# gildas-lormeau/zlib-streams-ts

Measured on AMD Instinct MI355X. Metric: uncompressed MB/s, deflate-raw L6, 4096x64KiB batch at 1/2/4/8 GPUs, higher is better.
Workload: dtype u8; 1 GPU; 4096 x 65536 B text-corpus streams split across the GPUs, deflate-raw level 6; global_streams=4096, streams_per_gpu=4096, stream_bytes=65536, level=6, format=deflate-raw, compressed_bytes=91855591, parallelism=dp1

## Files before the change

zlib-streams-ts_amd/csrc/deflate_parse.hip:

```cpp
#include <hip/hip_runtime.h>
#include <type_traits>
#include "zs_common.h"
#include "zs_kernels.h"
#include "zs_parse.h"

template <uint32_t SEG>
struct zs_seg_cfg {
  static constexpr uint32_t SPEC = (SEG + 260u + 3u) & ~3u;
  static constexpr uint32_t SYNC = SEG + 4u;
  static constexpr uint32_t FIX = SPEC;
  static constexpr uint32_t WORDS = SPEC + SYNC + FIX;
};
static_assert(zs_seg_cfg<ZS_PARSE_SEG>::WORDS == ZS_PARSE_SEG_WORDS, "scratch layout shared with capi.cpp");
static_assert(zs_seg_cfg<ZS_PARSE2W_SEG>::WORDS == ZS_PARSE2W_SEG_WORDS, "scratch layout shared with capi.cpp");
static_assert(zs_seg_cfg<ZS_PARSE4W_SEG>::WORDS == ZS_PARSE4W_SEG_WORDS, "scratch layout shared with capi.cpp");

#define ZS_WAVE_SYNC()                                   \
  do {                                                   \
    __builtin_amdgcn_fence(__ATOMIC_SEQ_CST, "workgroup"); \
    __builtin_amdgcn_wave_barrier();                     \
  } while (0)

struct zs_round_state {
  zs_pstate t;
  uint32_t total, last_sym;
};

template <uint32_t WIN>
struct zs_parse_win {
  uint4 m[WIN / 2][64];
};
template <>
struct zs_parse_win<0> {};

struct zs_seg_tab {
  uint32_t off[65];
  uint32_t nf[64];
  uint32_t from[64];
};

template <uint32_t WIN>
union zs_parse_lds {
  zs_parse_win<WIN> W;
  zs_seg_tab T;
};

static __device__ __forceinline__ uint32_t zs_sym_len(uint32_t v) {
  return (v & 0x80000000u) ? ((v >> 16) & 0xffu) + ZS_MIN_MATCH : 1u;
}
static __device__ __forceinline__ zs_pstate zs_read_state(const zs_pstate& x, uint32_t l) {
  zs_pstate r;
  r.p = (uint32_t)__builtin_amdgcn_readlane((int)x.p, (int)l);
  r.ma = (uint32_t)__builtin_amdgcn_readlane((int)x.ma, (int)l);
  r.ml = (uint32_t)__builtin_amdgcn_readlane((int)x.ml, (int)l);
  r.ms = (uint32_t)__builtin_amdgcn_readlane((int)x.ms, (int)l);
  return r;
}

#ifndef ZS_PARSE_PROF
#define ZS_PARSE_PROF 0
#endif
#if ZS_PARSE_PROF
__device__ unsigned long long zs_pp_stat[16];
extern "C" int zs_parse_stats(unsigned long long* out) {
  return (int)hipMemcpyFromSymbol(out, HIP_SYMBOL(zs_pp_stat), sizeof(zs_pp_stat));
}
#define PP_T(v) unsigned long long v = wall_clock64()
#define PP_ACC(i, v) do { if ((threadIdx.x & 63u) == 0) atomicAdd(&zs_pp_stat[i], wall_clock64() - v); } while (0)
#else
#define PP_T(v) do { } while (0)
#define PP_ACC(i, v) do { } while (0)
#endif

#define ZS_GATHER 16
#ifndef ZS_PARSE_WIN
#define ZS_PARSE_WIN 32
#endif


template <uint32_t WIN, uint32_t SEG, uint32_t NWV, bool DICT, bool FILT>
static __device__ __forceinline__ void zs_parse_body(zs_parse_win<WIN>& W, zs_seg_tab& T, zs_round_state& RS,
                                                     const uint8_t* __restrict__ in,
                                                     const uint64_t* __restrict__ in_off,
                                                     const uint32_t* __restrict__ in_len,
                                                     const uint64_t* __restrict__ pos_base,
                                                     const uint32_t* __restrict__ blk_base,
                                                     const uint2* __restrict__ mres, uint32_t* __restrict__ syms,
                                                     zs_block* __restrict__ blocks, zs_stream* __restrict__ streams,
                                                     uint32_t* __restrict__ scratch, int good, int lazy,
                                                     const uint32_t* __restrict__ dstart ZS_PAR_ARG) {
  using CF = zs_seg_cfg<SEG>;
  const int s = blockIdx.x;
  const uint32_t lane = threadIdx.x & 63u, wave = threadIdx.x >> 6;
  const uint32_t n = in_len[s];
  const uint32_t p0 = DICT ? dstart[s] : 0u;
  const uint8_t* src = in + in_off[s];
  const uint2* M = mres + pos_base[s];
  uint32_t* sy = syms + pos_base[s] + s;
  uint32_t* scr = scratch + (size_t)CF::WORDS * (pos_base[s] / SEG + s + 64u * wave);
  zs_block* blk = blocks + blk_base[s];
  const uint32_t nseg = (n - p0 + SEG - 1) / SEG;
  const bool aligned = ((uintptr_t)src & 3u) == 0;

  zs_pstate t = {p0, 0, ZS_MIN_MATCH - 1, 0};
  uint32_t total = 0;
  uint32_t last_sym = 0;
  if (NWV > 1) {
    if (threadIdx.x == 0) RS = {t, 0u, 0u};
    __syncthreads();
  }

  for (uint32_t sr = 0; sr < nseg; sr += 64u * NWV) {
    const uint32_t r0 = sr + 64u * wave;
    const uint32_t nr = r0 < nseg ? min(64u, nseg - r0) : 0u;
    const bool mine = lane < nr;
    const uint32_t a = mine ? p0 + (r0 + lane) * SEG : n, b = mine ? min(n, a + SEG) : n;
    uint32_t* spec = scr + (size_t)lane * CF::WORDS;
    uint32_t* sync = spec + CF::SPEC;
    uint32_t* fix = sync + CF::SYNC;

    PP_T(tA);
    zs_pstate st = {a, 0, ZS_MIN_MATCH - 1, 0};
    uint32_t cnt = 0;
    {
      uint32_t nsync = 0;
      uint4 sacc = make_uint4(0, 0, 0, 0), yacc = make_uint4(0, 0, 0, 0);
      auto step = [&](uint2 e, uint32_t lit) __attribute__((always_inline)) {
        if (st.ml == ZS_MIN_MATCH - 1) {
          const uint32_t y = ((st.p - a) << 17) | (st.ma << 16) | cnt, m = nsync & 3u;
          yacc.x = m == 0 ? y : yacc.x;
          yacc.y = m == 1 ? y : yacc.y;
          yacc.z = m == 2 ? y : yacc.z;
          yacc.w = m == 3 ? y : yacc.w;
          if (++nsync % 4 == 0) *reinterpret_cast<uint4*>(sync + nsync - 4) = yacc;
        }
        const uint32_t v = zs_parse_step<FILT>(st, e, lit, n, good, lazy ZS_PAR_PASS);
        if (v != ZS_NONE) {
          const uint32_t m = cnt & 3u;
          sacc.x = m == 0 ? v : sacc.x;
          sacc.y = m == 1 ? v : sacc.y;
          sacc.z = m == 2 ? v : sacc.z;
          sacc.w = m == 3 ? v : sacc.w;
          if (++cnt % 4 == 0) *reinterpret_cast<uint4*>(spec + cnt - 4) = sacc;
        }
      };
      if constexpr (WIN == 0) {
        while (st.p < b) {
          const uint32_t p = st.p;
          step(M[p], p > 0 ? src[p - 1] : 0u);
        }
      } else {
        constexpr uint32_t NP = WIN / 2;
        const uint32_t c = lane & (NP - 1u), tg = lane & ~(NP - 1u);
        const uint4* g = reinterpret_cast<const uint4*>(M);
        const uint32_t glast = ((n + 7u) >> 1) & ~3u;
        const uint32_t* s4 = reinterpret_cast<const uint32_t*>(src);
        const uint32_t slast = (n - 1u) >> 2;
        const uint32_t cw = (c + 1u) >> 1;
        for (uint64_t staging; (staging = __ballot(st.p < b)) != 0;) {
          const uint32_t w = st.p & ~3u;
          auto stage = [&](auto al) __attribute__((always_inline)) {
            constexpr bool AL = decltype(al)::value;
            uint4 mv[NP];
            uint32_t sv[NP];
            const uint32_t act = (uint32_t)(staging >> tg) & ((1u << NP) - 1u);
            uint32_t tb = tg << 2, c7 = c & 7u;
            asm volatile("" : "+v"(tb), "+v"(c7));
#pragma unroll
            for (uint32_t r = 0; r < NP; r++) sv[r] = (uint32_t)__builtin_amdgcn_ds_bpermute((int)(tb + 4u * r), (int)w);
#pragma unroll
            for (uint32_t r = 0; r < NP; r++) {
              if ((act >> r) & 1u) {
                const uint32_t wt = sv[r];
                mv[r] = g[min(wt / 2 + c, glast - 1u)];
                if constexpr (AL) {
                  sv[r] = s4[min(max(wt / 4 + cw, 1u) - 1u, slast)];
                } else {
                  uint16_t h = 0;
                  if (n > 1) __builtin_memcpy(&h, src + min(max(wt + 2u * c, 1u), n - 1u) - 1u, 2);
                  sv[r] = n > 1 ? (uint32_t)h | ((wt | c) == 0 ? 0x10000u : 0u) : src[0] | 0x10000u;
                }
              }
            }
#pragma unroll
            for (uint32_t r = 0; r < NP; r++) {
              uint32_t l0, l1;
              if constexpr (AL) {
                const uint32_t nx = (uint32_t)__builtin_amdgcn_update_dpp(0, (int)sv[r], 0x101, 0xf, 0xf, false);
                l0 = (c & 1u) ? (sv[r] >> 8) & 0xffu : sv[r] >> 24;
                l1 = (c & 1u) ? (sv[r] >> 16) & 0xffu : nx & 0xffu;
              } else {
                l0 = sv[r] & 0xffu;
                l1 = (sv[r] >> 16) ? l0 : (sv[r] >> 8) & 0xffu;
              }
              mv[r].x |= l0 << 25;
              mv[r].y |= (l0 >> 7) << 31;
              mv[r].z |= l1 << 25;
              mv[r].w |= (l1 >> 7) << 31;
              if ((act >> r) & 1u) W.m[c][tg + (r ^ c7)] = mv[r];
            }
          };
          if (aligned) stage(std::true_type{}); else stage(std::false_type{});
          while (st.p < b && st.p < w + WIN) {
            const uint32_t o = st.p - w;
            const uint2 e = reinterpret_cast<const uint2*>(&W.m[o >> 1][lane ^ ((o >> 1) & 7u)])[o & 1];
            step(e, (e.x >> 25) | ((e.y >> 31) << 7));
          }
        }
      }
      if (mine) {
        for (uint32_t i = nsync & ~3u; i < nsync; i++) sync[i] = (i & 3u) == 0 ? yacc.x : (i & 3u) == 1 ? yacc.y : yacc.z;
        for (uint32_t i = cnt & ~3u; i < cnt; i++) spec[i] = (i & 3u) == 0 ? sacc.x : (i & 3u) == 1 ? sacc.y : sacc.z;
        sync[nsync] = ZS_NONE;
        if (b == n && st.ma) spec[cnt++] = src[n - 1];
      }
    }

    PP_ACC(0, tA);
    uint32_t nf = 0, from = ZS_NONE, start = 0, R = 0, tot0 = 0;
    bool final_lit_r = false;
    for (uint32_t k = 0; k < NWV + (NWV > 1 ? 1u : 0u); k++) {
    if (NWV > 1) __syncthreads();
    if (nr != 0 && k == wave) {
    PP_T(tB);
    if (NWV > 1) {
      t = RS.t;
      total = RS.total;
    }
    zs_pstate after;
    auto catch_up = [&](zs_pstate c) __attribute__((always_inline)) {
      uint32_t si = 0, sv = sync[0];
      uint4 facc = make_uint4(0, 0, 0, 0);
      nf = 0;
      from = ZS_NONE;
      start = c.p - c.ma;
      while (c.p < b) {
        if (c.ml == ZS_MIN_MATCH - 1) {
          const uint32_t key = ((c.p - a) << 1) | c.ma;
          while ((sv >> 16) < key) sv = sync[++si];
          if ((sv >> 16) == key) { from = sv & 0xffffu; break; }
        }
        const uint32_t p = c.p;
        const uint32_t v = zs_parse_step<FILT>(c, M[p], p > 0 ? src[p - 1] : 0u, n, good, lazy ZS_PAR_PASS);
        if (v != ZS_NONE) {
          const uint32_t m = nf & 3u;
          facc.x = m == 0 ? v : facc.x;
          facc.y = m == 1 ? v : facc.y;
          facc.z = m == 2 ? v : facc.z;
          facc.w = m == 3 ? v : facc.w;
          if (++nf % 4 == 0) *reinterpret_cast<uint4*>(fix + nf - 4) = facc;
        }
      }
      for (uint32_t i = nf & ~3u; i < nf; i++) fix[i] = (i & 3u) == 0 ? facc.x : (i & 3u) == 1 ? facc.y : facc.z;
      if (from == ZS_NONE && b == n && c.ma) fix[nf++] = src[n - 1];
      after = from != ZS_NONE ? st : c;
    };
    {
      zs_pstate e;
      const int up = (int)((lane + 63u) & 63u);
      e.p = (uint32_t)__shfl((int)st.p, up, 64);
      e.ma = (uint32_t)__shfl((int)st.ma, up, 64);
      e.ml = (uint32_t)__shfl((int)st.ml, up, 64);
      e.ms = (uint32_t)__shfl((int)st.ms, up, 64);
      if (lane == 0) e = t;
      if (mine) catch_up(e);
    }
    for (uint32_t j = 0; j < nr; j++) {
      if (j > 0 && (uint32_t)__builtin_amdgcn_readlane((int)from, (int)(j - 1)) == ZS_NONE) {
        if (lane == j) catch_up(t);
      }
      t = zs_read_state(after, j);
    }

    const uint32_t run = mine ? nf + (from == ZS_NONE ? 0u : cnt - from) : 0u;
    uint32_t incl = run;
#pragma unroll
    for (int d = 1; d < 64; d <<= 1) {
      const uint32_t y = __shfl_up(incl, d, 64);
      if (lane >= (uint32_t)d) incl += y;
    }
    R = (uint32_t)__builtin_amdgcn_readlane((int)incl, 63);
    T.off[lane] = incl - run;
    if (lane == 63) T.off[64] = R;
    T.nf[lane] = nf;
    T.from[lane] = from;
    tot0 = total;
    final_lit_r = r0 + nr == nseg && t.ma != 0;
    total += R;
    if (NWV > 1 && lane == 0) {
      RS.t = t;
      RS.total = total;
    }
    PP_ACC(1, tB);
    }
    if (nr != 0 && k == wave + (NWV > 1 ? 1u : 0u)) {
    ZS_WAVE_SYNC();
    PP_T(tC);
    uint32_t js = 0, lastv = 0;
    for (uint32_t g0 = 0; g0 < R; g0 += 64 * ZS_GATHER) {
      uint32_t v[ZS_GATHER];
#pragma unroll
      for (int k = 0; k < ZS_GATHER; k++) {
        const uint32_t g = g0 + 64 * k + lane;
        v[k] = 0;
        if (g < R) {
          while (T.off[js + 1] <= g) js++;
          const uint32_t i = g - T.off[js], nfj = T.nf[js];
          const uint32_t* base = scr + (size_t)js * CF::WORDS;
          v[k] = i < nfj ? base[CF::SPEC + CF::SYNC + i] : base[T.from[js] + i - nfj];
        }
      }
#pragma unroll
      for (int k = 0; k < ZS_GATHER; k++) {
        const uint32_t g = g0 + 64 * k + lane;
        if (g < R) sy[tot0 + g] = v[k];
        if (g == R - 1) lastv = v[k];
      }
    }
    if (R) {
      last_sym = (uint32_t)__shfl((int)lastv, (int)((R - 1) & 63u), 64);
      if (NWV > 1 && lane == 0) RS.last_sym = last_sym;
    }

    PP_ACC(2, tC);
    PP_T(tD);
    const uint32_t unchecked = final_lit_r ? tot0 + R - 1 : ZS_NONE;
    for (uint32_t gi = (tot0 / ZS_P_SYM_END + 1) * ZS_P_SYM_END - 1; gi < tot0 + R; gi += ZS_P_SYM_END) {
      if (gi == unchecked) continue;
      const uint32_t g = gi - tot0;
      uint32_t j = 0;
      while (T.off[j + 1] <= g) j++;
      const uint32_t i = g - T.off[j], nfj = T.nf[j], fj = T.from[j];
      const uint32_t* base = scr + (size_t)j * CF::WORDS;
      uint32_t acc = 0, li = 0;
      for (uint32_t q = lane; q <= i; q += 64) {
        const uint32_t l = zs_sym_len(q < nfj ? base[CF::SPEC + CF::SYNC + q] : base[fj + q - nfj]);
        acc += l;
        li = q == i ? l : li;
      }
#pragma unroll
      for (int d = 32; d >= 1; d >>= 1) {
        acc += __shfl_xor(acc, d, 64);
        li += __shfl_xor(li, d, 64);
      }
      const uint32_t end = (uint32_t)__builtin_amdgcn_readlane((int)start, (int)j) + acc;
      if (lane == 0) {
        const uint32_t bi = (gi + 1) / ZS_P_SYM_END - 1;
        blk[bi].in_end = end;
        blk[bi].pad = zs_slides(end - li + 1, n ZS_PAR_PASS);
      }
    }
    PP_ACC(3, tD);
    ZS_WAVE_SYNC();
    }
    }
  }
  if (NWV > 1) {
    __syncthreads();
    if (wave != 0) return;
    t = RS.t;
    total = RS.total;
    last_sym = RS.last_sym;
  }

  PP_T(tE);
  const bool final_lit = nseg > 0 && t.ma != 0;
  const uint32_t checked = final_lit ? total - 1 : total;
  const uint32_t nflush = checked / ZS_P_SYM_END;
  const uint32_t v_last = total == 0 ? 0u : final_lit ? n - 1 : n - zs_sym_len(last_sym) + 1;
  const uint32_t final_slides = zs_slides(v_last, n ZS_PAR_PASS);
  ZS_WAVE_SYNC();
  for (uint32_t b0 = 0; b0 <= nflush; b0 += 64) {
    const uint32_t b = b0 + lane;
    zs_block k;
    if (b <= nflush) {
      const uint32_t in_start = b == 0 ? p0 : blk[b - 1].in_end;
      const uint32_t in_end = b < nflush ? blk[b].in_end : n;
      const uint32_t slides = b < nflush ? blk[b].pad : final_slides;
      k.sym_start = b * ZS_P_SYM_END;
      k.sym_count = b < nflush ? ZS_P_SYM_END : total - nflush * ZS_P_SYM_END;
      k.in_start = in_start;
      k.in_end = in_end;
      k.type = 0; k.hdr_bits = 0; k.data_bits = 0; k.pad = 0; k.bit_off = 0; k.bit_end = 0;
      k.last = (b == nflush ? 1u : 0u) | ((uint64_t)in_start < ZS_P_W_ULL * slides ? 2u : 0u);
    }
    ZS_WAVE_SYNC();
    if (b <= nflush) blk[b] = k;
    ZS_WAVE_SYNC();
  }
  if (lane == 0) {
    streams[s].nsym = total;
    streams[s].nblk = nflush + 1;
  }
  PP_ACC(4, tE);
#if ZS_PARSE_PROF
  if (lane == 0) atomicAdd(&zs_pp_stat[5], 1ull);
#endif
}

#if ZS_PAR_BUILD
#define ZS_PARSE_KERNEL(name, WIN, SEG, NWV)                                                                        \
  __global__ __launch_bounds__(64 * NWV) void name##_par(                                                            \
      const uint8_t* __restrict__ in, const uint64_t* __restrict__ in_off, const uint32_t* __restrict__ in_len,     \
      const uint64_t* __restrict__ pos_base, const uint32_t* __restrict__ blk_base, const uint2* __restrict__ mres,  \
      uint32_t* __restrict__ syms, zs_block* __restrict__ blocks, zs_stream* __restrict__ streams,                  \
      uint32_t* __restrict__ scratch, int good, int lazy, zs_kpar kp) {                                             \
    __shared__ zs_parse_lds<WIN> U[NWV];                                                                            \
    __shared__ zs_round_state RS;                                                                                   \
    const uint32_t w_ = threadIdx.x >> 6;                                                                           \
    zs_parse_body<WIN, SEG, NWV, false, false>(U[w_].W, U[w_].T, RS, in, in_off, in_len, pos_base, blk_base, mres,  \
                                               syms, blocks, streams, scratch, good, lazy, nullptr, kp);            \
  }
#else
#define ZS_PARSE_KERNEL(name, WIN, SEG, NWV)                                                                        \
  __global__ __launch_bounds__(64 * NWV) void name(                                                                  \
      const uint8_t* __restrict__ in, const uint64_t* __restrict__ in_off, const uint32_t* __restrict__ in_len,     \
      const uint64_t* __restrict__ pos_base, const uint32_t* __restrict__ blk_base, const uint2* __restrict__ mres,  \
      uint32_t* __restrict__ syms, zs_block* __restrict__ blocks, zs_stream* __restrict__ streams,                  \
      uint32_t* __restrict__ scratch, int good, int lazy) {                                                         \
    __shared__ zs_parse_lds<WIN> U[NWV];                                                                            \
    __shared__ zs_round_state RS;                                                                                   \
    const uint32_t w_ = threadIdx.x >> 6;                                                                           \
    zs_parse_body<WIN, SEG, NWV, false, false>(U[w_].W, U[w_].T, RS, in, in_off, in_len, pos_base, blk_base, mres, syms,   \
                                        blocks, streams, scratch, good, lazy, nullptr);                             \
  }                                                                                                                  \
  __global__ __launch_bounds__(64 * NWV) void name##_dict(                                                           \
      const uint8_t* __restrict__ in, const uint64_t* __restrict__ in_off, const uint32_t* __restrict__ in_len,     \
      const uint64_t* __restrict__ pos_base, const uint32_t* __restrict__ blk_base, const uint2* __restrict__ mres,  \
      uint32_t* __restrict__ syms, zs_block* __restrict__ blocks, zs_stream* __restrict__ streams,                  \
      uint32_t* __restrict__ scratch, int good, int lazy, const uint32_t* __restrict__ dstart) {                    \
    __shared__ zs_parse_lds<WIN> U[NWV];                                                                            \
    __shared__ zs_round_state RS;                                                                                   \
    const uint32_t w_ = threadIdx.x >> 6;                                                                           \
    zs_parse_body<WIN, SEG, NWV, true, false>(U[w_].W, U[w_].T, RS, in, in_off, in_len, pos_base, blk_base, mres,  \
                                              syms, blocks, streams, scratch, good, lazy, dstart);                  \
  }                                                                                                                  \
  __global__ __launch_bounds__(64 * NWV) void name##_filt(                                                           \
      const uint8_t* __restrict__ in, const uint64_t* __restrict__ in_off, const uint32_t* __restrict__ in_len,     \
      const uint64_t* __restrict__ pos_base, const uint32_t* __restrict__ blk_base, const uint2* __restrict__ mres,  \
      uint32_t* __restrict__ syms, zs_block* __restrict__ blocks, zs_stream* __restrict__ streams,                  \
      uint32_t* __restrict__ scratch, int good, int lazy) {                                                         \
    __shared__ zs_parse_lds<WIN> U[NWV];                                                                            \
    __shared__ zs_round_state RS;                                                                                   \
    const uint32_t w_ = threadIdx.x >> 6;                                                                           \
    zs_parse_body<WIN, SEG, NWV, false, true>(U[w_].W, U[w_].T, RS, in, in_off, in_len, pos_base, blk_base, mres,  \
                                              syms, blocks, streams, scratch, good, lazy, nullptr);                 \
  }
#endif
ZS_PARSE_KERNEL(zs_k_parse, ZS_PARSE_WIN, ZS_PARSE_SEG, 1)
ZS_PARSE_KERNEL(zs_k_parse_2w, ZS_PARSE_WIN, ZS_PARSE2W_SEG, 2)
ZS_PARSE_KERNEL(zs_k_parse_4w, ZS_PARSE_WIN, ZS_PARSE4W_SEG, 4)
```

zlib-streams-ts_amd/csrc/zs_parse.h:

```cpp
#pragma once
#include <hip/hip_runtime.h>
#include <stdint.h>
#include "zs_common.h"
#include "zs_par.h"

#define ZS_NONE 0xffffffffu

struct zs_pstate {
  uint32_t p, ma, ml, ms;
};

template <bool FILT = false>
static __device__ __forceinline__ uint32_t zs_parse_step(zs_pstate& st, uint2 e, uint32_t lit, uint32_t n, int good,
                                                         int lazy ZS_PAR_ARG) {
  const uint32_t p = st.p, pl = st.ml, pm = st.ms;
  const bool nil = ((e.x & 0x8000u) != 0) & (p >= ZS_P_SLIDE_AT) & (((p - ZS_P_SLIDE_AT) & ZS_P_WMASK) == 0) &
                   (n - p < (uint32_t)ZS_MIN_LOOKAHEAD);
  const bool search = (((e.x >> 16) & 0x1ffu) != 0) & (pl < (uint32_t)lazy) & !nil;
  const uint32_t u = pl >= (uint32_t)good ? e.y : e.x;
  const uint32_t L = (u >> 16) & 0x1ffu, D = u & 0x7fffu;
  const bool take = search & (L > pl);
  const uint32_t ms = take ? p - D : pm;
  const bool too_far = FILT ? L <= 5u : (L == ZS_MIN_MATCH) & (D > ZS_TOO_FAR);
  const uint32_t ml = (take & !too_far) ? L : ZS_MIN_MATCH - 1;
  const bool emit = (pl >= ZS_MIN_MATCH) & (ml <= pl);
  const uint32_t sym = 0x80000000u | ((pl - ZS_MIN_MATCH) << 16) | (p - 1 - pm);
  const uint32_t ret = emit ? sym : (st.ma ? lit : ZS_NONE);
  st.p = emit ? p + pl - 1 : p + 1;
  st.ma = emit ? 0u : 1u;
  st.ml = emit ? ZS_MIN_MATCH - 1 : ml;
  st.ms = ms;
  return ret;
}

static __device__ __forceinline__ uint32_t zs_slides(uint32_t v, uint32_t n ZS_PAR_ARG) {
  if (n <= v + 261u) return v >= ZS_P_SLIDE_AT ? (v - ZS_P_SLIDE_AT) / ZS_P_W + 1u : 0u;
  return v >= ZS_P_SLIDE_AT + 1u ? (v - ZS_P_SLIDE_AT - 1u) / ZS_P_W + 1u : 0u;
}
```

Baseline: 23270 MB/s.

## Stage parse outputs in LDS window slots and flush them as coalesced uint4 stores

The speculative lazy-match parse loop no longer packs symbols and sync records into register accumulators with per-element selects and data-dependent global uint4 stores. Instead, each step writes its symbol and sync word into the already-consumed slots of the per-lane LDS window. After every window it flushes them to global memory in wave-uniform loops of uint4 stores, carrying up to three leftover words between windows. The nil-slide check is also hoisted to one precomputed position per window, and the WIN==0 path is dropped. This should cut divergent global stores and per-step ALU, at the cost of extra LDS traffic and flush loops.

```diff
diff --git a/zlib-streams-ts_amd/csrc/deflate_parse.hip b/zlib-streams-ts_amd/csrc/deflate_parse.hip
--- a/zlib-streams-ts_amd/csrc/deflate_parse.hip
+++ b/zlib-streams-ts_amd/csrc/deflate_parse.hip
@@ -28,10 +28,11 @@
 
 template <uint32_t WIN>
 struct zs_parse_win {
+  static_assert(WIN >= 16 && WIN % 16 == 0, "the stage's groups of WIN / 2 lanes swizzle eight columns");
   uint4 m[WIN / 2][64];
 };
-template <>
-struct zs_parse_win<0> {};
+typedef uint2 __attribute__((may_alias)) zs_win_u2;
+typedef uint32_t __attribute__((may_alias)) zs_win_u1;
 
 struct zs_seg_tab {
   uint32_t off[65];
@@ -124,32 +125,31 @@
     uint32_t cnt = 0;
     {
       uint32_t nsync = 0;
-      uint4 sacc = make_uint4(0, 0, 0, 0), yacc = make_uint4(0, 0, 0, 0);
-      auto step = [&](uint2 e, uint32_t lit) __attribute__((always_inline)) {
-        if (st.ml == ZS_MIN_MATCH - 1) {
-          const uint32_t y = ((st.p - a) << 17) | (st.ma << 16) | cnt, m = nsync & 3u;
-          yacc.x = m == 0 ? y : yacc.x;
-          yacc.y = m == 1 ? y : yacc.y;
-          yacc.z = m == 2 ? y : yacc.z;
-          yacc.w = m == 3 ? y : yacc.w;
-          if (++nsync % 4 == 0) *reinterpret_cast<uint4*>(sync + nsync - 4) = yacc;
+      char* const wl = reinterpret_cast<char*>(&W);
+      uint32_t cs0 = 0, cs1 = 0, cs2 = 0, ck0 = 0, ck1 = 0, ck2 = 0;
+      auto flush = [&](uint32_t* dst, uint32_t n0, uint32_t k, uint32_t word, uint32_t& c0, uint32_t& c1,
+                       uint32_t& c2) __attribute__((always_inline)) {
+        const uint32_t r = n0 & 3u, G = zs_collect_whole(r, k);
+        uint32_t* const d4 = dst + (n0 & ~3u);
+        auto at = [&](uint32_t q) __attribute__((always_inline)) {
+          return *reinterpret_cast<const zs_win_u1*>(wl + zs_win_off((q - r) & (WIN - 1u), lane) + word);
+        };
+        for (uint32_t g = 0; __ballot(g < G) != 0; g++) {
+          uint32_t v0 = at(4u * g), v1 = at(4u * g + 1u), v2 = at(4u * g + 2u);
+          const uint32_t v3 = at(4u * g + 3u);
+          if (g == 0) {
+            v0 = r > 0 ? c0 : v0;
+            v1 = r > 1 ? c1 : v1;
+            v2 = r > 2 ? c2 : v2;
+          }
+          if (g < G) *reinterpret_cast<uint4*>(d4 + 4u * g) = make_uint4(v0, v1, v2, v3);
         }
-        const uint32_t v = zs_parse_step<FILT>(st, e, lit, n, good, lazy ZS_PAR_PASS);
-        if (v != ZS_NONE) {
-          const uint32_t m = cnt & 3u;
-          sacc.x = m == 0 ? v : sacc.x;
-          sacc.y = m == 1 ? v : sacc.y;
-          sacc.z = m == 2 ? v : sacc.z;
-          sacc.w = m == 3 ? v : sacc.w;
-          if (++cnt % 4 == 0) *reinterpret_cast<uint4*>(spec + cnt - 4) = sacc;
-        }
+        const uint32_t t0 = at(4u * G), t1 = at(4u * G + 1u), t2 = at(4u * G + 2u);
+        c0 = ((G == 0) & (r > 0)) ? c0 : t0;
+        c1 = ((G == 0) & (r > 1)) ? c1 : t1;
+        c2 = ((G == 0) & (r > 2)) ? c2 : t2;
       };
-      if constexpr (WIN == 0) {
-        while (st.p < b) {
-          const uint32_t p = st.p;
-          step(M[p], p > 0 ? src[p - 1] : 0u);
-        }
-      } else {
+      {
         constexpr uint32_t NP = WIN / 2;
         const uint32_t c = lane & (NP - 1u), tg = lane & ~(NP - 1u);
         const uint4* g = reinterpret_cast<const uint4*>(M);
@@ -201,16 +201,29 @@
             }
           };
           if (aligned) stage(std::true_type{}); else stage(std::false_type{});
+          const uint32_t cnt0 = cnt;
+          uint32_t ny = 0;
+          const uint32_t p_nil = zs_parse_nil_pos(w, WIN, n, ZS_P_SLIDE_AT, ZS_P_W);
           while (st.p < b && st.p < w + WIN) {
-            const uint32_t o = st.p - w;
-            const uint2 e = reinterpret_cast<const uint2*>(&W.m[o >> 1][lane ^ ((o >> 1) & 7u)])[o & 1];
-            step(e, (e.x >> 25) | ((e.y >> 31) << 7));
+            const uint32_t p = st.p;
+            const uint2 e = *reinterpret_cast<const zs_win_u2*>(wl + zs_win_off(p - w, lane));
+            const uint32_t y = ((p - a) << 17) | (st.ma << 16) | cnt;
+            const bool ysync = st.ml == ZS_MIN_MATCH - 1;
+            const bool nil = ((e.x & 0x8000u) != 0) & (p == p_nil);
+            const uint32_t v = zs_parse_step<FILT>(st, e, (e.x >> 25) | ((e.y >> 31) << 7), nil, good, lazy);
+            *reinterpret_cast<zs_win_u1*>(wl + zs_win_off(ny, lane) + 4u) = y;
+            *reinterpret_cast<zs_win_u1*>(wl + zs_win_off(zs_collect_slot(cnt, cnt0), lane)) = v;
+            ny += ysync ? 1u : 0u;
+            cnt += v != ZS_NONE ? 1u : 0u;
           }
+          flush(spec, cnt0, cnt - cnt0, 0u, cs0, cs1, cs2);
+          flush(sync, nsync, ny, 4u, ck0, ck1, ck2);
+          nsync += ny;
         }
       }
       if (mine) {
-        for (uint32_t i = nsync & ~3u; i < nsync; i++) sync[i] = (i & 3u) == 0 ? yacc.x : (i & 3u) == 1 ? yacc.y : yacc.z;
-        for (uint32_t i = cnt & ~3u; i < cnt; i++) spec[i] = (i & 3u) == 0 ? sacc.x : (i & 3u) == 1 ? sacc.y : sacc.z;
+        for (uint32_t i = nsync & ~3u; i < nsync; i++) sync[i] = (i & 3u) == 0 ? ck0 : (i & 3u) == 1 ? ck1 : ck2;
+        for (uint32_t i = cnt & ~3u; i < cnt; i++) spec[i] = (i & 3u) == 0 ? cs0 : (i & 3u) == 1 ? cs1 : cs2;
         sync[nsync] = ZS_NONE;
         if (b == n && st.ma) spec[cnt++] = src[n - 1];
       }
diff --git a/zlib-streams-ts_amd/csrc/zs_parse.h b/zlib-streams-ts_amd/csrc/zs_parse.h
--- a/zlib-streams-ts_amd/csrc/zs_parse.h
+++ b/zlib-streams-ts_amd/csrc/zs_parse.h
@@ -1,6 +1,27 @@
 #pragma once
+#include <stdint.h>
+
+#if defined(__HIPCC__)
+#define ZS_PARSE_FN static __host__ __device__ __forceinline__
+#else
+#define ZS_PARSE_FN static inline
+#endif
+
+
+ZS_PARSE_FN uint32_t zs_win_off(uint32_t k, uint32_t lane) {
+  const uint32_t k8 = k << 3;
+  return ((k << 9) & ~0x200u) | (k8 & 8u) | ((lane << 4) ^ (k8 & 0x70u));
+}
+ZS_PARSE_FN uint32_t zs_collect_slot(uint32_t count, uint32_t count0) { return count - count0; }
+ZS_PARSE_FN uint32_t zs_collect_whole(uint32_t r, uint32_t k) { return (r + k) >> 2; }
+
+ZS_PARSE_FN uint32_t zs_parse_nil_pos(uint32_t w, uint32_t win, uint32_t n, uint32_t slide_at, uint32_t w_size) {
+  const uint32_t c = w + ((slide_at - w) & (w_size - 1u));
+  return ((c - w < win) & (c >= slide_at) & (n - c < 262u)) ? c : 0xffffffffu;
+}
+
+#if defined(__HIPCC__)
 #include <hip/hip_runtime.h>
-#include <stdint.h>
 #include "zs_common.h"
 #include "zs_par.h"
 
@@ -11,11 +32,9 @@
 };
 
 template <bool FILT = false>
-static __device__ __forceinline__ uint32_t zs_parse_step(zs_pstate& st, uint2 e, uint32_t lit, uint32_t n, int good,
-                                                         int lazy ZS_PAR_ARG) {
+static __device__ __forceinline__ uint32_t zs_parse_step(zs_pstate& st, uint2 e, uint32_t lit, bool nil, int good,
+                                                         int lazy) {
   const uint32_t p = st.p, pl = st.ml, pm = st.ms;
-  const bool nil = ((e.x & 0x8000u) != 0) & (p >= ZS_P_SLIDE_AT) & (((p - ZS_P_SLIDE_AT) & ZS_P_WMASK) == 0) &
-                   (n - p < (uint32_t)ZS_MIN_LOOKAHEAD);
   const bool search = (((e.x >> 16) & 0x1ffu) != 0) & (pl < (uint32_t)lazy) & !nil;
   const uint32_t u = pl >= (uint32_t)good ? e.y : e.x;
   const uint32_t L = (u >> 16) & 0x1ffu, D = u & 0x7fffu;
@@ -25,15 +44,26 @@
   const uint32_t ml = (take & !too_far) ? L : ZS_MIN_MATCH - 1;
   const bool emit = (pl >= ZS_MIN_MATCH) & (ml <= pl);
   const uint32_t sym = 0x80000000u | ((pl - ZS_MIN_MATCH) << 16) | (p - 1 - pm);
-  const uint32_t ret = emit ? sym : (st.ma ? lit : ZS_NONE);
-  st.p = emit ? p + pl - 1 : p + 1;
+  const uint32_t deferred = st.ma ? lit : ZS_NONE;
+  const uint32_t p_emit = p + pl - 1, p_lit = p + 1;
+  const uint32_t ret = emit ? sym : deferred;
+  st.p = emit ? p_emit : p_lit;
   st.ma = emit ? 0u : 1u;
   st.ml = emit ? ZS_MIN_MATCH - 1 : ml;
   st.ms = ms;
   return ret;
+}
+template <bool FILT = false>
+static __device__ __forceinline__ uint32_t zs_parse_step(zs_pstate& st, uint2 e, uint32_t lit, uint32_t n, int good,
+                                                         int lazy ZS_PAR_ARG) {
+  const uint32_t p = st.p;
+  const bool nil = ((e.x & 0x8000u) != 0) & (p >= ZS_P_SLIDE_AT) & (((p - ZS_P_SLIDE_AT) & ZS_P_WMASK) == 0) &
+                   (n - p < (uint32_t)ZS_MIN_LOOKAHEAD);
+  return zs_parse_step<FILT>(st, e, lit, nil, good, lazy);
 }
 
 static __device__ __forceinline__ uint32_t zs_slides(uint32_t v, uint32_t n ZS_PAR_ARG) {
   if (n <= v + 261u) return v >= ZS_P_SLIDE_AT ? (v - ZS_P_SLIDE_AT) / ZS_P_W + 1u : 0u;
   return v >= ZS_P_SLIDE_AT + 1u ? (v - ZS_P_SLIDE_AT - 1u) / ZS_P_W + 1u : 0u;
 }
+#endif
```

After: 23350 MB/s, median of 6. Within noise of the previous version (+0.4%).
